# jakubbober/discrete-curvature-rewiring

Hardware: AMD Instinct MI355X
Metric: SDRF iterations/sec (higher is better)
Workload: dtype f64; 1 GPU; S100k: preferential-attachment graph N=100000 m=10 E=999900 (PCG64 seed 12345), Balanced Forman curvature, full recompute every iteration, remove_edges=True, tau=163.0, removal_bound=0.95; parallelism=single GPU

## Files before the change

discrete-curvature-rewiring_amd/csrc/dcr_bfc_h2.hip:

```cpp
#include <algorithm>
#include <climits>
#include <cstdio>
#include <cstdlib>
#include <cstring>
#include <vector>

#include "dcr_bfc_common.h"

namespace dcr {

constexpr unsigned H2_EMPTY = 0xFFFFFFFFu;
constexpr unsigned H2_NBR = 0x80000000u;
constexpr int H2_CLASSES = 5;
constexpr int H2_WB = 4;
__device__ inline unsigned h2_rec_t(int T, int deg) { return (unsigned)T | ((unsigned)deg << 16); }
static_assert(H2_MAXDEG < 65536, "record packing");
constexpr int H2_SMALL_DEG = 64;
#ifndef H2_Q
#define H2_Q 2
#endif
#ifndef H2_QL
#define H2_QL 2
#endif
constexpr int H2_QCAP = 128;
// ... 943 lines not shown
    int pln = sc->pln;
#pragma unroll 1
    while (true) {
        const int i = lcur + lane;
        const unsigned item = i < ls.n ? ls.items[i] : 0xFFFFFFFFu;
        const bool mine = i < ls.n && (int)(item >> 19) == bidx;
        const int cnt = __popcll(__ballot(mine));
        if (cnt == 0) break;
        const int s = (int)(item & 0x1FFFu), r = (int)((item >> 13) & 63u);
        const unsigned w = mine ? t.key[s] : 0u;
        h2_settle<L1, EXS>(t, sc, mine, mine ? s : -1, r, w, pln, tk, al, tbase);
        lcur += cnt;
        if (cnt < 64) break;
    }
    if (lane == 0) sc->pln = pln;
    h2_wave_sync();
}

__device__ inline void h2_batch_begin(const H2Tasks tk, H2Alloc &al, H2Scratch *sc, int k, int &tbase, int &trow, int rev = -1) {
    const int lane = threadIdx.x & 63;
    const unsigned long long below = (1ull << lane) - 1ull;
    sc->rowT[lane] = 0;
    sc->rowPos[lane] = 0;
    sc->rowMx[lane] = 0;
    sc->rowRev[lane] = rev;
    if (lane == 0) sc->pln = 0;
    int dummy_c, dummy_p;
    const unsigned long long rows = __ballot(k >= 0);
    if (!h2_pool_reserve(tk, al, __popcll(rows), 0, 0, tbase, dummy_c, dummy_p)) tbase = -1;
    trow = __popcll(rows & below);
    sc->trank[lane] = (unsigned char)trow;
    trow += tbase;
}

template <int L1, int EXS, bool PARTS>
__device__ inline void h2_batch_end(const View &g, const H2Tasks tk, H2Alloc &al, int u, int2 ru, int i, int k, int2 rk, int tbase,
                                    int trow, int part, const H2Tab t, H2Scratch *sc, uint4 *rec, const unsigned *items = nullptr,
                                    int ifrom = 0, int ito = 0) {
    const int lane = threadIdx.x & 63;
    int T = sc->rowT[lane], pos = sc->rowPos[lane], mx = sc->rowMx[lane];
    const int rev = sc->rowRev[lane];
    bool listed = tbase >= 0 && k >= 0 && T > 0 && pos > 0 && rev >= 0 && rev < g.cap_total;
    int ep;
    const int Pn = h2_prefix(listed ? T : 0, ep);
    int p0 = 0;
    if (Pn > 0) {
        int dummy_t, dummy_c;
        if (!h2_pool_reserve(tk, al, 0, 0, Pn, dummy_t, dummy_c, p0)) listed = false;
    }
    if (__ballot(listed) != 0ull) {
        const int pln = sc->pln;
        if (pln <= H2_PLCAP) {
            sc->poff[lane] = listed ? p0 + ep : -1;
            h2_wave_sync();
            for (int j = lane; j < pln; j += 64) {
                const int r = sc->plr[j];
                if (sc->poff[r] >= 0) tk.part[atomicAdd(&sc->poff[r], 1)] = (int32_t)sc->plt[j];
            }
            h2_wave_sync();
        } else if (items) {
            sc->poff[lane] = listed ? p0 + ep : -1;
            h2_wave_sync();
            for (int j = ifrom + lane; j < ito; j += 64) {
                const unsigned item = items[j];
                const int s2 = (int)(item & 0x1FFFu), r = (int)((item >> 13) & 63u);
                if ((h2_cnt_get(t.cnt, s2) & 0x8000u) && sc->poff[r] >= 0) tk.part[atomicAdd(&sc->poff[r], 1)] = (int32_t)t.key[s2];
            }
            h2_wave_sync();
        } else {
            const bool shortrow = listed && rk.y <= H2_SHORT_ROW;
            if (shortrow) h2_partners_short<L1, EXS>(g, tk, u, rk, p0 + ep, T, t);
            unsigned long long todo = __ballot(listed && !shortrow);
            while (todo) {
                const int l = __ffsll((long long)todo) - 1;
                todo &= todo - 1;
                const int2 rv = make_int2(__shfl(rk.x, l), __shfl(rk.y, l));
                h2_partners_of_row<L1, EXS>(g, tk, u, rv, __shfl(p0 + ep, l), __shfl(T, l), t);
            }
        }
    }
    if (tbase >= 0 && k >= 0) {
        tk.task[trow] = listed ? make_uint4((unsigned)(ru.x + i), (unsigned)(p0 + ep), (unsigned)T, (unsigned)u | tk.retry_flag)
                               : make_uint4(0u, 0u, H2_TASK_VOID, 0u);
    }
    if (listed) {
        pos = 0;
        mx = 0;
    }
    if (k >= 0) {
        const int64_t slot = (int64_t)ru.x + i;
        if (rev < 0 || rev >= g.cap_total) {
            row_ok(g, make_int2(-1, rev), 33, u, k);
        } else if (!PARTS) {
            rec[slot] = make_uint4((unsigned)pos, (unsigned)mx, h2_rec_t(T, ru.y), (unsigned)rev);
        } else {
            unsigned *r4 = reinterpret_cast<unsigned *>(rec + slot);
            if (pos) atomicAdd(&r4[0], (unsigned)pos);
            if (mx) atomicMax(&r4[1], (unsigned)mx);
            if (part == 0) {
                r4[2] = h2_rec_t(T, ru.y);
                r4[3] = (unsigned)rev;
            }
        }
    }
}

constexpr int H2_JOIN_MAXM = 256;
__device__ inline int h2_probe_partners(const H2EdgeSet es, int w, const int32_t *pt, int np);

template <int L1, int EXS, int NW>
__device__ inline bool h2_join_prepare(const View &g, const H2Tab t, int2 ru, const H2List &ls) {
    constexpr int NT = 64 * NW, PER = EXS / NT;
    static_assert(PER >= 2 && PER % 2 == 0, "a thread owns whole cursor words");
    static_assert(EXS / 2 <= (1 << L1) / 32, "the cursors fit B1");
    static_assert(NW * H2_ITEMS < 65536 && EXS <= 8192, "16-bit cursors, 13-bit slots");
    const int tid = (int)threadIdx.x, lane = tid & 63, wid = tid >> 6;
    unsigned *cur = t.b1;
    int n[PER], sum = 0, most = 0;
#pragma unroll
    for (int q = 0; q < PER; ++q) {
        const unsigned c16 = h2_cnt_get(t.cnt, tid * PER + q);
        n[q] = ((c16 & 0x8000u) || c16 < 2u) ? 0 : (int)c16;
        sum += n[q];
        most = n[q] > most ? n[q] : most;
    }
    if (__syncthreads_or(most > H2_JOIN_MAXM)) return false;
    int excl;
    const int wtot = h2_prefix(sum, excl);
    if (lane == 0) t.wsum[wid] = wtot;
    __syncthreads();
    int off = excl;
    for (int w = 0; w < wid; ++w) off += t.wsum[w];
#pragma unroll
    for (int q = 0; q < PER; q += 2) {
        const unsigned lo = (unsigned)off;
        off += n[q];
        const unsigned hi = (unsigned)off;
        off += n[q + 1];
        cur[(tid * PER + q) >> 1] = lo | (hi << 16);
    }
    __syncthreads();
    for (int base = 0; base < ls.n; base += 64) {
        const int j = base + lane;
        if (j >= ls.n) continue;
        const unsigned item = ls.items[j];
        const int s = (int)(item & 0x1FFFu), r = (int)((item >> 13) & 63u), b = (int)(item >> 19);
        const unsigned c16 = h2_cnt_get(t.cnt, s);
        if ((c16 & 0x8000u) || c16 < 2u) continue;
        const int row = (b * 64 + r) * NW + wid;
        if (row >= ru.y) {
            row_ok(g, make_int2(-1, row), 44, ru.y, (int)item);
            continue;
        }
        const int v = g.col[ru.x + row];
        const unsigned old = atomicAdd(&cur[s >> 1], 1u << ((s & 1) * 16));
        const int p = (int)((old >> ((s & 1) * 16)) & 0xFFFFu);
        if (p < NW * H2_ITEMS) ls.srt[p] = v;
        else row_ok(g, make_int2(-1, p), 45, s, (int)c16);
    }
    __syncthreads();
    return true;
}

template <int L1, int EXS, int NW, bool PARTS>
__device__ inline void h2_batch_join(const View &g, const H2Tasks tk, H2Alloc &al, int u, int2 ru, int i, int k, int2 rk, int part,
                                     const H2Tab t, H2Scratch *sc, uint4 *rec, const H2List &ls, int &lcur, int bidx, int rev) {
    const int lane = threadIdx.x & 63;
    sc->rowT[lane] = 0;
    sc->rowPos[lane] = 0;
    sc->rowMx[lane] = 0;
    sc->rowRev[lane] = rev;
    if (lane == 0) sc->pln = 0;
    h2_wave_sync();
    const int lfrom = lcur;
#pragma unroll 1
    while (true) {
        const int j = lcur + lane;
        const unsigned item = j < ls.n ? ls.items[j] : 0xFFFFFFFFu;
        const bool mine = j < ls.n && (int)(item >> 19) == bidx;
        const int cnt = __popcll(__ballot(mine));
        if (cnt == 0) break;
        if (mine && (h2_cnt_get(t.cnt, (int)(item & 0x1FFFu)) & 0x8000u)) atomicAdd(&sc->rowT[(item >> 13) & 63u], 1);
        lcur += cnt;
        if (cnt < 64) break;
    }
    h2_wave_sync();
    const unsigned *cur = t.b1;
#pragma unroll 1
    for (int base = lfrom; base < lcur; base += 64) {
        const int j = base + lane;
        const bool have = j < lcur;
        const unsigned item = have ? ls.items[j] : 0u;
        const int s = (int)(item & 0x1FFFu), r = (int)((item >> 13) & 63u);
        const int vr = __shfl(k, r);
        if (!have) continue;
        const unsigned c16 = h2_cnt_get(t.cnt, s);
        if (c16 & 0x8000u) continue;
        const int m = (int)(c16 & 0x7FFFu);
        int c = m - 1;
        if (c <= 0) continue;
        if (sc->rowT[r] > 0 && vr >= 0) {
            const int end = (int)((cur[s >> 1] >> ((s & 1) * 16)) & 0xFFFFu);
            if (end >= m && end <= NW * H2_ITEMS) {
                c -= h2_probe_partners(tk.es, vr, ls.srt + (end - m), m);
            } else {
                row_ok(g, make_int2(-1, end), 46, s, m);
                c = 0;
            }
        }
        if (c > 0) {
            atomicAdd(&sc->rowPos[r], 1);
            atomicMax(&sc->rowMx[r], c);
        }
    }
    h2_wave_sync();
    h2_batch_end<L1, EXS, PARTS>(g, tk, al, u, ru, i, k, rk, -1, 0, part, t, sc, rec);
}

template <int L1, int EXS, int NW, bool PARTS, int PHASE>
__device__ inline void h2_stream(const View &g, const H2Tasks tk, H2Alloc &al, int u, int2 ru, int part, int nparts,
                                 const H2Tab t, H2Scratch *sc, uint4 *rec, int k0, int2 rk0, H2List &ls) {
    const int lane = threadIdx.x & 63;
    const int wid = (int)(threadIdx.x >> 6);
    int qn = 0;
    int lcur = 0;
    if (PHASE == 0 && ru.y > 64 * NW * H2_REV_BATCHES) ls.over = true;
    for (int base = 0; base < ru.y; base += 64 * NW) {
        const int i = base + lane * NW + wid;
        int k = k0;
        int2 rk = rk0;
        if (base > 0) {
            k = -1;
            rk = make_int2(0, 0);
            if (i < ru.y) {
                k = g.col[ru.x + i];
                if (k >= 0 && k < g.n && k != u) {
                    rk = g.rowinfo[k];
                    if (!row_ok(g, rk, 32, k, u)) rk = make_int2(0, 0);
                } else {
                    k = -1;
                }
            }
        }
        const int np = rk.y > 0 ? ((rk.x + rk.y + 3) >> 2) - (rk.x >> 2) : 0;
        int poff_lane;
        const int P = h2_prefix(np, poff_lane);
        if (P == 0) continue;
        const int bidx = base / (64 * NW);
        int tbase = -1, trow = 0;
        if (PHASE == 2 && !ls.over) {
            if (ls.join) {
                h2_batch_join<L1, EXS, NW, PARTS>(g, tk, al, u, ru, i, k, rk, part, t, sc, rec, ls, lcur, bidx, ls.revs[bidx * 64 + lane]);
                h2_wave_sync();
                continue;
            }
            h2_batch_begin(tk, al, sc, k, tbase, trow, ls.revs[bidx * 64 + lane]);
            h2_wave_sync();
            const int lfrom = lcur;
            h2_settle_items<L1, EXS>(t, sc, ls, lcur, bidx, tk, al, tbase);
            h2_batch_end<L1, EXS, PARTS>(g, tk, al, u, ru, i, k, rk, tbase, trow, part, t, sc, rec, ls.items, lfrom, lcur);
            h2_wave_sync();
            continue;
        }
        if (PHASE == 0 && !ls.over) ls.revs[bidx * 64 + lane] = -1;
        sc->desc[lane] = rk;
        sc->poff[lane] = poff_lane;
        if (lane == 0) sc->poff[64] = P;
        if (PHASE == 2) h2_batch_begin(tk, al, sc, k, tbase, trow);
        h2_wave_sync();
        const bool listing = PHASE == 1 && !ls.over;
        auto flags = [&](const int4 w, unsigned vm, int r, int a) -> unsigned {
            const unsigned kk[4] = {(unsigned)w.x, (unsigned)w.y, (unsigned)w.z, (unsigned)w.w};
            const unsigned isu = h2_eq4(kk, (unsigned)u) & vm;
            if (PHASE == 2 && isu) sc->rowRev[r] = a + __ffs((int)isu) - 1;
            if (listing && isu) ls.revs[bidx * 64 + r] = a + __ffs((int)isu) - 1;
            unsigned valid = vm & ~isu;
            if (PARTS && PHASE != 2 && !listing) {
#pragma unroll
                for (int jj = 0; jj < 4; ++jj)
                    if (h2_part(kk[jj], nparts) != part) valid &= ~(1u << jj);
            }
            if (PHASE == 0) {
                h2_mark4<L1>(t.b1, t.b2, kk, valid);
                return 0u;
            }
            return h2_again4<L1>(t.b2, kk, valid);
        };
        h2_for_pieces_queued<(PARTS ? H2_QL : H2_Q)>(g.col, sc->desc, sc->poff, poff_lane, P, qn, flags,
                             [&](int idx, unsigned key, int r) {
                                 sc->qw[idx] = key;
                                 if (PHASE != 0) sc->qr[idx] = (unsigned char)r;
                                 if (PHASE == 1) sc->qb[idx] = (unsigned char)bidx;
                             },
                             [&]() { h2_drain<L1, EXS, PHASE, PARTS>(t, sc, qn, tk, al, tbase, ls, part, nparts); });
        if (PHASE == 2) {
            h2_drain<L1, EXS, PHASE, PARTS>(t, sc, qn, tk, al, tbase, ls, part, nparts);
            h2_batch_end<L1, EXS, PARTS>(g, tk, al, u, ru, i, k, rk, tbase, trow, part, t, sc, rec);
        }
        h2_wave_sync();
    }
    if (qn > 0) h2_drain<L1, EXS, PHASE, PARTS>(t, sc, qn, tk, al, -1, ls, part, nparts);
}

constexpr int H2_NPB = 12;
template <int L1, int EXS, int NW, bool PARTS>
__device__ inline bool h2_node_fast(const View &g, const H2Tasks tk, H2Alloc &al, int u, int2 ru, int part, int nparts,
                                    const H2Tab t, H2Scratch *sc, uint4 *rec, bool &ok, H2List &ls) {
    const int tid = (int)threadIdx.x, lane = tid & 63, wid = tid >> 6;
    constexpr int NT = 64 * NW, NP = H2_NPB;
    const unsigned long long below = (1ull << lane) - 1ull;
    if (ru.y > 64 * NW) return false;
    const int i = lane * NW + wid;
    int k = -1;
    int2 rk = make_int2(0, 0);
    if (i < ru.y) {
        k = g.col[ru.x + i];
        if (k >= 0 && k < g.n && k != u) {
            rk = g.rowinfo[k];
            if (!row_ok(g, rk, 32, k, u)) rk = make_int2(0, 0);
        } else {
            k = -1;
        }
    }
    const int np = rk.y > 0 ? ((rk.x + rk.y + 3) >> 2) - (rk.x >> 2) : 0;
    int poff_lane;
    const int P = h2_prefix(np, poff_lane);
    if (__syncthreads_or(P > 64 * NP)) return false;
    {
        uint4 *z = reinterpret_cast<uint4 *>(t.b1);
        constexpr int NZ = ((1 << L1) / 32 + (1 << (L1 - 2)) / 32) / 4;
        for (int j = tid; j < NZ; j += NT) z[j] = make_uint4(0u, 0u, 0u, 0u);
        uint4 *k4 = reinterpret_cast<uint4 *>(t.key);
        for (int j = tid; j < EXS / 4; j += NT) k4[j] = make_uint4(H2_EMPTY, H2_EMPTY, H2_EMPTY, H2_EMPTY);
        uint4 *c4 = reinterpret_cast<uint4 *>(t.cnt);
        for (int j = tid; j < EXS / 8; j += NT) c4[j] = make_uint4(0u, 0u, 0u, 0u);
        if (tid == 0) *t.full = 0;
    }
    sc->desc[lane] = rk;
    sc->poff[lane] = poff_lane;
    if (lane == 0) sc->poff[64] = P;
    h2_wave_sync();
    int4 w[NP];
    unsigned long long meta[NP];
#pragma unroll
    for (int q = 0; q < NP; ++q) {
        const int j = 64 * q + lane;
        w[q] = make_int4(0, 0, 0, 0);
        meta[q] = 0ull;
        const int jf = 64 * q, jl = jf + 63 < P ? jf + 63 : P - 1;
        if (jf >= P) continue;
        const int r = h2_piece_row(sc->poff, poff_lane, j < P ? j : jl, jf, jl);
        if (j < P) {
            const int2 d = sc->desc[r];
            const int a = (d.x & ~3) + 4 * (j - sc->poff[r]);
            w[q] = load_piece(g.col, a);
            meta[q] = (unsigned long long)h2_piece_mask(a, d.x, d.x + d.y) | ((unsigned long long)r << 8) | ((unsigned long long)(unsigned)a << 16);
        }
    }
    __syncthreads();
    if (k >= 0) {
        const int sl = h2_insert<EXS>(t.key, (unsigned)k);
        if (sl < 0) *t.full = 1;
        else h2_cnt_flag(t.cnt, sl);
        h2_seed<L1>(t.b1, t.b2, (unsigned)k);
    }
    __syncthreads();
#pragma unroll
    for (int q = 0; q < NP; ++q) {
        if (64 * q >= P) continue;
        const unsigned kk[4] = {(unsigned)w[q].x, (unsigned)w[q].y, (unsigned)w[q].z, (unsigned)w[q].w};
        unsigned valid = (unsigned)meta[q] & 0xFu & ~h2_eq4(kk, (unsigned)u);
        if (PARTS) {
#pragma unroll
            for (int jj = 0; jj < 4; ++jj)
                if (h2_part(kk[jj], nparts) != part) valid &= ~(1u << jj);
        }
        meta[q] |= (unsigned long long)valid << 4;
        h2_mark4<L1>(t.b1, t.b2, kk, valid);
    }
    __syncthreads();
    int qn = 0, tbase = -1, trow = 0;
    sc->rowRev[lane] = -1;
    h2_wave_sync();
    {
        unsigned fl[NP];
#pragma unroll
        for (int q = 0; q < NP; ++q) {
            fl[q] = 0u;
            if (64 * q >= P) continue;
            const unsigned kk[4] = {(unsigned)w[q].x, (unsigned)w[q].y, (unsigned)w[q].z, (unsigned)w[q].w};
            const unsigned valid = (unsigned)(meta[q] >> 4) & 0xFu;
            const unsigned isu = h2_eq4(kk, (unsigned)u) & (unsigned)meta[q] & 0xFu;
            if (isu) sc->rowRev[(int)((meta[q] >> 8) & 0xFFull)] = (int)(meta[q] >> 16) + __ffs((int)isu) - 1;
            fl[q] = h2_again4<L1>(t.b2, kk, valid);
        }
#pragma unroll 1
        while (true) {
            bool stop = false;
#pragma unroll
            for (int q = 0; q < NP; ++q) {
                if (64 * q >= P) continue;
                const unsigned kk[4] = {(unsigned)w[q].x, (unsigned)w[q].y, (unsigned)w[q].z, (unsigned)w[q].w};
#pragma unroll
                for (int jj = 0; jj < 4; ++jj) {
                    const bool p = (fl[q] >> jj) & 1u;
                    const unsigned long long m = __ballot(p);
                    if (m == 0ull) continue;
                    if (stop || qn + __popcll(m) > H2_QCAP) {
                        stop = true;
                        continue;
                    }
                    if (p) {
                        const int idx = qn + __popcll(m & below);
                        sc->qw[idx] = kk[jj];
                        sc->qr[idx] = (unsigned char)((meta[q] >> 8) & 0xFFull);
                        sc->qb[idx] = 0;
                        fl[q] &= ~(1u << jj);
                    }
                    qn += __popcll(m);
                }
            }
            if (qn > 0) h2_drain<L1, EXS, 1, PARTS>(t, sc, qn, tk, al, -1, ls, part, nparts);
            if (!stop) break;
        }
    }
    __syncthreads();
    ok = *t.full == 0;
    ls.join = !__syncthreads_or(ls.over) && ok;
    if (ls.join) ls.join = h2_join_prepare<L1, EXS, NW>(g, t, ru, ls);
    if (ls.join) {
        int lcur = 0;
        const int myrev = sc->rowRev[lane];
        h2_wave_sync();
        h2_batch_join<L1, EXS, NW, PARTS>(g, tk, al, u, ru, i, k, rk, part, t, sc, rec, ls, lcur, 0, myrev);
    } else if (ok) {
        if (tid == 0) atomicAdd(&tk.res->h2_fallback, 1);
        if (!ls.over) {
            int lcur = 0;
            const int myrev = sc->rowRev[lane];
            h2_wave_sync();
            h2_batch_begin(tk, al, sc, k, tbase, trow, myrev);
            h2_wave_sync();
            h2_settle_items<L1, EXS>(t, sc, ls, lcur, 0, tk, al, tbase);
            h2_batch_end<L1, EXS, PARTS>(g, tk, al, u, ru, i, k, rk, tbase, trow, part, t, sc, rec, ls.items, 0, lcur);
        } else {
            h2_stream<L1, EXS, NW, PARTS, 2>(g, tk, al, u, ru, part, nparts, t, sc, rec, k, rk, ls);
        }
    }
    __syncthreads();
    return true;
}

template <int L1, int EXS, int NW, bool PARTS>
__device__ inline bool h2_node(const View &g, const H2Tasks tk, H2Alloc &al, int u, int2 ru, int part, int nparts,
                               const H2Tab t, H2Scratch *sc, uint4 *rec, H2List &ls) {
    const int tid = (int)threadIdx.x;
    constexpr int NT = 64 * NW;
    if constexpr (!PARTS) {
        bool ok_fast = true;
        if (h2_node_fast<L1, EXS, NW, PARTS>(g, tk, al, u, ru, part, nparts, t, sc, rec, ok_fast, ls)) return ok_fast;
    }
    int k0 = -1;
    int2 rk0 = make_int2(0, 0);
    {
        const int i0 = (tid & 63) * NW + (tid >> 6);
        if (i0 < ru.y) {
            k0 = g.col[ru.x + i0];
            if (k0 >= 0 && k0 < g.n && k0 != u) {
                rk0 = g.rowinfo[k0];
                if (!row_ok(g, rk0, 32, k0, u)) rk0 = make_int2(0, 0);
            } else {
                k0 = -1;
            }
        }
    }
    {
        uint4 *z = reinterpret_cast<uint4 *>(t.b1);
        constexpr int NZ = ((1 << L1) / 32 + (1 << (L1 - 2)) / 32) / 4;
        for (int i = tid; i < NZ; i += NT) z[i] = make_uint4(0u, 0u, 0u, 0u);
        uint4 *k4 = reinterpret_cast<uint4 *>(t.key);
        for (int i = tid; i < EXS / 4; i += NT) k4[i] = make_uint4(H2_EMPTY, H2_EMPTY, H2_EMPTY, H2_EMPTY);
        uint4 *c4 = reinterpret_cast<uint4 *>(t.cnt);
        for (int i = tid; i < EXS / 8; i += NT) c4[i] = make_uint4(0u, 0u, 0u, 0u);
        if (tid == 0) *t.full = 0;
    }
    __syncthreads();
    for (int i = tid; i < ru.y; i += NT) {
        const int k = g.col[ru.x + i];
        if (k >= 0 && k < g.n && k != u) {
            const int s = h2_insert<EXS>(t.key, (unsigned)k);
            if (s < 0) *t.full = 1;
            else h2_cnt_flag(t.cnt, s);
            h2_seed<L1>(t.b1, t.b2, (unsigned)k);
        }
    }
    __syncthreads();
    h2_stream<L1, EXS, NW, PARTS, 0>(g, tk, al, u, ru, part, nparts, t, sc, rec, k0, rk0, ls);
    __syncthreads();
    h2_stream<L1, EXS, NW, PARTS, 1>(g, tk, al, u, ru, part, nparts, t, sc, rec, k0, rk0, ls);
    __syncthreads();
    const bool ok = *t.full == 0;
    ls.join = !__syncthreads_or(ls.over) && ok;
    if (ls.join) ls.join = h2_join_prepare<L1, EXS, NW>(g, t, ru, ls);
    if (!ls.join && ok && tid == 0) atomicAdd(&tk.res->h2_fallback, 1);
    if (ok) h2_stream<L1, EXS, NW, PARTS, 2>(g, tk, al, u, ru, part, nparts, t, sc, rec, k0, rk0, ls);
    __syncthreads();
    return ok;
}

template <int L1, int EXS, int NW, bool PARTS>
__global__ void __launch_bounds__(64 * NW) __attribute__((amdgpu_waves_per_eu(3))) k_h2_block(View g, H2Tasks tk, const int4 *units, const int32_t *count, int64_t unit_cap,
                                                       uint4 *rec, H2Retry rt, int is_retry) {
    __shared__ __attribute__((aligned(16))) unsigned bits[(1 << L1) / 32 + (1 << (L1 - 2)) / 32];
    __shared__ __attribute__((aligned(16))) unsigned key[EXS];
    __shared__ __attribute__((aligned(16))) unsigned cnt[EXS / 2];
    __shared__ H2Scratch sc_all[NW];
    __shared__ int full;
    __shared__ int wsum[NW];
    const int wid = threadIdx.x >> 6;
    const int total = *count;
    if (total < 0 || total > unit_cap) {
        row_ok(g, make_int2(-1, total), 37, 0, 0);
        return;
    }
    const H2Tab t{bits, bits + (1 << L1) / 32, key, cnt, &full, wsum};
    H2Alloc al;
    for (int64_t it = blockIdx.x; it < total; it += gridDim.x) {
        const int4 un = units[it];
        const int u = un.x;
        const int nparts = PARTS ? (int)((unsigned)un.y >> 16) : 1, part = PARTS ? (un.y & 0xFFFF) : 0;
        bool ok = u >= 0 && u < g.n && nparts >= 1 && part < nparts;
        int2 ru = make_int2(0, 0);
        if (ok) {
            ru = g.rowinfo[u];
            ok = row_ok(g, ru, 38, u, (int)it) && ru.y > 0 && ru.y <= H2_MAXDEG;
        }
        if (!ok) continue;
        H2List ls = h2_list_of(tk.lists, NW);
        const bool unit_ok = h2_node<L1, EXS, NW, PARTS>(g, tk, al, u, ru, part, nparts, t, &sc_all[wid], rec, ls);
        if (!unit_ok) {
            if (threadIdx.x == 0) {
                if (is_retry) {
                    rt.res->h2_status = 1;
                    atomicAdd(&rt.res->h2_failed[5], 1);
                } else {
                    h2_retry_push(rt, u, ru.y, PARTS ? 4 : 3);
                }
            }
        }
    }
    h2_void_candidates(tk, al.c_cur, al.c_end);
    h2_void_tasks(tk, al.t_cur, al.t_end);
}

__device__ inline int h2_probe_partners(const H2EdgeSet es, int w, const int32_t *pt, int np) {
    int found = 0;
    for (int j = 0; j < np; j += 8) {
        int tt[8];
#pragma unroll
        for (int q = 0; q < 8; ++q) tt[q] = j + q < np ? pt[j + q] : -1;
        unsigned long long key[8], k0[8], h[8];
        unsigned bw[8], bb[8];
#pragma unroll
        for (int q = 0; q < 8; ++q) {
            key[q] = h2_edge_key(w, tt[q] < 0 ? w : tt[q]);
            bb[q] = h2_bloom_bit(key[q], es.bloom_bits);
            bw[q] = es.bloom[bb[q] >> 5];
        }
#pragma unroll
        for (int q = 0; q < 8; ++q) {
            const bool maybe = tt[q] >= 0 && ((bw[q] >> (bb[q] & 31u)) & 1u);
            h[q] = h2_eset_slot(key[q], es.bits);
            k0[q] = maybe ? es.tab[h[q]] : H2_ESET_EMPTY;
        }
#pragma unroll
        for (int q = 0; q < 8; ++q) {
            bool hit = k0[q] == key[q];
            if (!hit && k0[q] != H2_ESET_EMPTY) hit = h2_eset_has(es, w, tt[q]);
            found += hit ? 1 : 0;
        }
    }
    return found;
}

__global__ void __launch_bounds__(256) k_h2_triangles(H2EdgeSet es, H2Tasks tk, uint4 *rec, const int32_t *status, int second) {
    const int cand_now = *tk.n_cand;
    const int first = second ? *tk.n_done : 0;
    const int total = cand_now < tk.cand_cap ? cand_now : (int)tk.cand_cap;
    if (!second && blockIdx.x == 0 && threadIdx.x == 0) *tk.n_done = cand_now;
    if (*status != 0) return;
    if (total <= first || first < 0) return;
    const int lane = threadIdx.x & 63;
    for (int64_t base = first + (((int64_t)blockIdx.x * 256 + threadIdx.x) & ~63ll); base < total; base += (int64_t)gridDim.x * 256) {
        const int64_t i = base + lane;
        int c = 0;
        unsigned slot = 0xFFFFFFFFu;
        if (i < total) {
            const int4 cd = tk.cand[i];
            const uint4 ts = (cd.z >= 0 && cd.z < tk.task_cap) ? tk.task[cd.z] : make_uint4(0u, 0u, H2_TASK_VOID, 0u);
            const bool skip = ts.z == H2_TASK_VOID || (!(ts.w & 0x80000000u) && ((unsigned)tk.weight[ts.w & 0x7FFFFFFFu] & 0x80000000u));
            if (!skip) {
                slot = ts.x;
                c = cd.y - h2_probe_partners(es, cd.x, tk.part + ts.y, (int)ts.z);
            }
        }
        const unsigned prev = (unsigned)__shfl_up((int)slot, 1);
        const bool head = lane == 0 || prev != slot;
        const unsigned long long heads = __ballot(head);
        const int seg = __popcll(heads & ((2ull << lane) - 1ull));
        int n = c > 0 ? 1 : 0, mx = c > 0 ? c : 0;
#pragma unroll
        for (int off = 1; off < 64; off <<= 1) {
            const int s2 = __shfl_up(seg, off), n2 = __shfl_up(n, off), m2 = __shfl_up(mx, off);
            if (lane >= off && s2 == seg) {
                n += n2;
                mx = m2 > mx ? m2 : mx;
            }
        }
        const bool tail = lane == 63 || ((heads >> (lane + 1)) & 1ull);
        if (tail && n > 0 && slot != 0xFFFFFFFFu) {
            unsigned *r4 = reinterpret_cast<unsigned *>(rec + slot);
            atomicAdd(&r4[0], (unsigned)n);
            atomicMax(&r4[1], (unsigned)mx);
        }
    }
}

__global__ void __launch_bounds__(256) k_h2_weight(View g, int32_t *weight) {
    const int64_t s = (int64_t)blockIdx.x * 256 + threadIdx.x;
    const int lane = threadIdx.x & 63;
    int u = -1, val = 0;
    if (s < g.cap_total) {
        const int us = g.slot_row[s];
        const int v = g.col[s];
        const bool uok = us >= 0 && us < g.n, vok = v >= 0 && v < g.n;
        const int2 ru = g.rowinfo[uok ? us : 0];
        const int dv = g.rowinfo[vok ? v : 0].y;
        if (uok) {
            u = us;
            if (vok && s >= ru.x && (int)(s - ru.x) < ru.y) val = dv;
        }
    }
#pragma unroll
    for (int off = 1; off < 64; off <<= 1) {
        const int t = __shfl_up(val, off), uu = __shfl_up(u, off);
        if (lane >= off && uu == u) val += t;
    }
    const int un = __shfl_down(u, 1);
    if (u >= 0 && val > 0 && (lane == 63 || un != u)) atomicAdd(&weight[u], val);
}

constexpr int H2_NB = H2_CLASSES * H2_WB;
__device__ inline void h2_clear_result(DevResult *res, int tid, int half, bool flags_cleared) {
    if (tid == 0 && flags_cleared) res->touched_n = 0;
    if (tid < 8) res->misc[tid] = 0;
    if (tid < H2_NB) {
        res->h2_bucket[half][tid] = 0;
        res->h2_fill[half][tid] = 0;
    }
    if (tid < H2_CLASSES) res->h2_count[tid] = 0;
    if (tid == 0) {
        res->h2_status = 0;
        res->h2_retry = 0;
        for (int p = 0; p < 2; ++p) res->h2_ntask[p] = res->h2_ncand[p] = res->h2_npart[p] = res->h2_ncand_done[p] = 0;
        for (int c = 0; c < 6; ++c) res->h2_failed[c] = 0;
        res->h2_fallback = 0;
        res->flag_too_big = 0;
    }
}
struct H2Lists {
    int4 *units[H2_CLASSES];
    int64_t cap[H2_CLASSES];
};
constexpr int H2_PLAN_THREADS = 1024;

__device__ inline void h2_classify(int d, int S, int &cls, int &wb, int &nparts) {
    nparts = 1;
    int lo = 0;
    if (d <= H2_SMALL_DEG && S <= h2_maxw(2)) {
        cls = S <= h2_maxw(0) ? 0 : S <= h2_maxw(1) ? 1 : 2;
        lo = cls == 0 ? 0 : h2_maxw(cls - 1);
        wb = (int)((int64_t)(S - lo) * H2_WB / (h2_maxw(cls) - lo + 1));
    } else if (S <= h2_maxw(3) && d + S / 4 <= h2_keycap(3)) {
        cls = 3;
        wb = S < 2048 ? 0 : S < 4096 ? 1 : S < 6144 ? 2 : 3;
    } else {
        cls = 4;
        nparts = h2_parts_for(d, S, false);
        wb = S < 16384 ? 0 : S < 32768 ? 1 : S < 65536 ? 2 : 3;
    }
    if (wb > H2_WB - 1) wb = H2_WB - 1;
    if (wb < 0) wb = 0;
}

template <int PHASE>
__global__ void __launch_bounds__(H2_PLAN_THREADS) k_h2_plan(View g, int32_t *weight, H2Lists L, DevResult *res, int parity, int head,
                                                             unsigned *dirty_words, int64_t n_dirty_words, uint4 *rec) {
    __shared__ int blk_count[H2_NB];
    __shared__ int blk_base[H2_NB];
    const int u = blockIdx.x * H2_PLAN_THREADS + threadIdx.x;
    const int lane = threadIdx.x & 63;
    if (threadIdx.x < H2_NB) blk_count[threadIdx.x] = 0;
    __syncthreads();
    int bkt = -1, cls = -1, wb = 0, nparts = 0;
    int2 ru = make_int2(0, 0);
    if (u < g.n) {
        ru = g.rowinfo[u];
        const int d = ru.y;
        const int wraw = weight[u];
        if (PHASE == 0 && wraw < 0) weight[u] = wraw & 0x7FFFFFFF;
        if (d > 0 && d <= H2_MAXDEG) {
            h2_classify(d, wraw & 0x7FFFFFFF, cls, wb, nparts);
            bkt = cls * H2_WB + wb;
        }
    }
    if (PHASE == 0 && head) {
        const int64_t stride = (int64_t)gridDim.x * H2_PLAN_THREADS;
        for (int64_t i = (int64_t)blockIdx.x * H2_PLAN_THREADS + threadIdx.x; i < n_dirty_words; i += stride) dirty_words[i] = 0u;
        if (blockIdx.x == 0) h2_clear_result(res, (int)threadIdx.x, 1 - parity, n_dirty_words > 0);
    }
    const int nunits = bkt < 0 ? 0 : nparts;
    int my_off = 0;
    for (int b = 0; b < H2_NB; ++b) {
        const unsigned long long m = __ballot(bkt == b);
        if (m == 0) continue;
        int incl = bkt == b ? nunits : 0;
        for (int off = 1; off < 64; off <<= 1) {
            const int t = __shfl_up(incl, off);
            if (lane >= off) incl += t;
        }
        const int tot = __shfl(incl, 63);
        int wave_off = 0;
        if (lane == 0) wave_off = atomicAdd(&blk_count[b], tot);
        wave_off = __shfl(wave_off, 0);
        if (bkt == b) my_off = wave_off + incl - nunits;
    }
    __syncthreads();
    if (threadIdx.x < H2_NB) {
        const int b = threadIdx.x, c = blk_count[b];
        if (PHASE == 0) {
            if (c) atomicAdd(&res->h2_bucket[parity][b], c);
        } else {
            int before = 0;
            for (int h = b + 1; h < H2_NB; ++h)
                if (h / H2_WB == b / H2_WB) before += res->h2_bucket[parity][h];
            blk_base[b] = before + (c ? atomicAdd(&res->h2_fill[parity][b], c) : 0);
        }
    }
    if (PHASE == 0) return;
    if (blockIdx.x == 0 && threadIdx.x >= 64 && threadIdx.x < 64 + H2_CLASSES) {
        const int c = (int)threadIdx.x - 64;
        int64_t tot = 0;
        for (int b = c * H2_WB; b < (c + 1) * H2_WB; ++b) tot += res->h2_bucket[parity][b];
        if (tot > (c == 0 ? L.cap[0] : c == 1 ? L.cap[1] : c == 2 ? L.cap[2] : c == 3 ? L.cap[3] : L.cap[4])) {
            res->h2_status = 1;
            tot = 0;
        }
        res->h2_count[c] = (int)tot;
    }
    __syncthreads();
    if (bkt >= 0) {
        const int64_t first = (int64_t)blk_base[bkt] + my_off;
        int4 *dst = cls == 0 ? L.units[0] : cls == 1 ? L.units[1] : cls == 2 ? L.units[2] : cls == 3 ? L.units[3] : L.units[4];
        const int64_t cap = cls == 0 ? L.cap[0] : cls == 1 ? L.cap[1] : cls == 2 ? L.cap[2] : cls == 3 ? L.cap[3] : L.cap[4];
        static_assert(H2_CLASSES == 5, "the selects above list the classes");
        if (nparts <= 65535 && first >= 0 && first + nunits <= cap) {
            for (int j = 0; j < nunits; ++j) dst[first + j] = make_int4(u, (nparts << 16) | j, ru.x, ru.y);
        } else if (nparts > 65535) {
            res->h2_status = 1;
        }
    }
    if (!head) return;
    const int64_t piece = (int64_t)((lane >> 3) * (H2_PLAN_THREADS / 64) + (int)(threadIdx.x >> 6)) * gridDim.x + blockIdx.x;
    const int64_t z = piece * 8 + (lane & 7);
    int2 rz = make_int2(0, 0);
    bool is_split = false;
    if (z < g.n) {
        rz = g.rowinfo[z];
        if (rz.y > 0 && rz.y <= H2_MAXDEG) {
            int zc, zb, zp;
            h2_classify(rz.y, weight[z] & 0x7FFFFFFF, zc, zb, zp);
            is_split = zc == 4;
        }
    }
    unsigned long long split = __ballot(is_split);
    while (split) {
        const int src = __ffsll((long long)split) - 1;
        split &= split - 1ull;
        const int2 rs = make_int2(__shfl(rz.x, src), __shfl(rz.y, src));
        if (!row_ok(g, rs, 42, __shfl((int)z, src), -1)) continue;
        for (int i = lane; i < rs.y; i += 64) rec[(int64_t)rs.x + i] = make_uint4(0u, 0u, 0u, 0u);
    }
}

__global__ void __launch_bounds__(256) k_h2_clear(DevResult *res, int32_t *weight, int64_t n, unsigned *dirty_words, int64_t n_dirty_words) {
    for (int64_t i = (int64_t)blockIdx.x * 256 + threadIdx.x; i < n; i += (int64_t)gridDim.x * 256) weight[i] = 0;
    for (int64_t i = (int64_t)blockIdx.x * 256 + threadIdx.x; i < n_dirty_words; i += (int64_t)gridDim.x * 256) dirty_words[i] = 0u;
    if (blockIdx.x != 0) return;
    h2_clear_result(res, (int)threadIdx.x, 0, n_dirty_words > 0);
    h2_clear_result(res, (int)threadIdx.x, 1, n_dirty_words > 0);
}

__global__ void __launch_bounds__(256) k_h2_retry_zero(View g, const int4 *units, const int32_t *count, int64_t unit_cap, uint4 *rec) {
    const int total = *count;
    if (total <= 0 || total > unit_cap) return;
    for (int64_t it = blockIdx.x; it < total; it += gridDim.x) {
        const int4 un = units[it];
        if ((un.y & 0xFFFF) != 0 || un.x < 0 || un.x >= g.n) continue;
        const int2 ru = g.rowinfo[un.x];
        if (!row_ok(g, ru, 42, un.x, (int)it)) continue;
        for (int i = threadIdx.x; i < ru.y; i += 256) rec[(int64_t)ru.x + i] = make_uint4(0u, 0u, 0u, 0u);
    }
}

#ifndef H2_FINAL_Q
#define H2_FINAL_Q 1
#endif
#ifndef H2_FINAL_BLOCKS
#define H2_FINAL_BLOCKS 1024
#endif
__global__ void __launch_bounds__(256) k_h2_final(View g, const uint4 *rec, double *curv, const int32_t *status, Ext *part_min,
                                                  Ext *part_max, const int32_t *retry_count, int when, const int32_t *fallback_count,
                                                  int tri_stage) {
    if (when == 0 && *retry_count > 0) {
        if (blockIdx.x == 0 && threadIdx.x == 0) atomicCAS(const_cast<int32_t *>(status), 0, 3);
        return;
    }
    if (tri_stage == 0 && *fallback_count > 0) {
        if (blockIdx.x == 0 && threadIdx.x == 0) atomicCAS(const_cast<int32_t *>(status), 0, 4);
        return;
    }
    double lo_v = 0.0, hi_v = 0.0;
    int lo_s = -1, hi_s = -1;
    const bool live = *status == 0;
    const int64_t stride = (int64_t)gridDim.x * 256;
    constexpr int Q = H2_FINAL_Q;
    for (int64_t s0 = (int64_t)blockIdx.x * 256 + threadIdx.x; live && s0 < g.cap_total; s0 += Q * stride) {
        int u[Q], v[Q];
        uint4 a[Q];
        bool want[Q];
#pragma unroll
        for (int q = 0; q < Q; ++q) {
            const int64_t s = s0 + q * stride;
            const bool in = s < g.cap_total;
            u[q] = in ? g.slot_row[s] : -1;
            v[q] = in ? g.col[s] : -1;
            a[q] = in ? rec[s] : make_uint4(0u, 0u, 0u, 0u);
        }
        int2 ru[Q];
        int dv[Q], rcol[Q], rrow[Q];
        uint4 b[Q];
// ... 306 lines not shown
```

Before: 1119 iterations/sec.

## Software-pipeline unit and neighbour-head loads across block-loop iterations in H2 kernel

Prefetches the next two work units, plus the first-hop neighbour index and row info for the next unit, while the current unit is processed. Row offset and degree carried inside the unit record let the kernel skip a dependent rowinfo load. It also uses readfirstlane to keep unit fields uniform in scalar registers. The goal is to hide the global-memory latency of the dependent col/rowinfo chain at the start of each unit, at the cost of extra live registers and reliance on units carrying valid row info in z/w.

```diff
diff --git a/discrete-curvature-rewiring_amd/csrc/dcr_bfc_h2.hip b/discrete-curvature-rewiring_amd/csrc/dcr_bfc_h2.hip
--- a/discrete-curvature-rewiring_amd/csrc/dcr_bfc_h2.hip
+++ b/discrete-curvature-rewiring_amd/csrc/dcr_bfc_h2.hip
@@ -1269,26 +1269,34 @@
     if (qn > 0) h2_drain<L1, EXS, PHASE, PARTS>(t, sc, qn, tk, al, -1, ls, part, nparts);
 }
 
+template <int NW>
+__device__ inline int h2_head_k(const View &g, int2 ru) {
+    const int i0 = (int)(threadIdx.x & 63) * NW + (int)(threadIdx.x >> 6);
+    return i0 < ru.y ? g.col[ru.x + i0] : -1;
+}
+__device__ inline int2 h2_head_rk(const View &g, int u, int k) {
+    return (k >= 0 && k < g.n && k != u) ? g.rowinfo[k] : make_int2(0, 0);
+}
+template <int NW>
+__device__ inline void h2_head_check(const View &g, int u, int2 ru, int &k, int2 &rk) {
+    const int i0 = (int)(threadIdx.x & 63) * NW + (int)(threadIdx.x >> 6);
+    if (i0 >= ru.y || k < 0 || k >= g.n || k == u) {
+        k = -1;
+        rk = make_int2(0, 0);
+    } else if (!row_ok(g, rk, 32, k, u)) {
+        rk = make_int2(0, 0);
+    }
+}
+
 constexpr int H2_NPB = 12;
-template <int L1, int EXS, int NW, bool PARTS>
+template <int L1, int EXS, int NW, bool PARTS, typename Mid>
 __device__ inline bool h2_node_fast(const View &g, const H2Tasks tk, H2Alloc &al, int u, int2 ru, int part, int nparts,
-                                    const H2Tab t, H2Scratch *sc, uint4 *rec, bool &ok, H2List &ls) {
+                                    const H2Tab t, H2Scratch *sc, uint4 *rec, bool &ok, H2List &ls, int k, int2 rk, Mid mid) {
     const int tid = (int)threadIdx.x, lane = tid & 63, wid = tid >> 6;
     constexpr int NT = 64 * NW, NP = H2_NPB;
     const unsigned long long below = (1ull << lane) - 1ull;
     if (ru.y > 64 * NW) return false;
     const int i = lane * NW + wid;
-    int k = -1;
-    int2 rk = make_int2(0, 0);
-    if (i < ru.y) {
-        k = g.col[ru.x + i];
-        if (k >= 0 && k < g.n && k != u) {
-            rk = g.rowinfo[k];
-            if (!row_ok(g, rk, 32, k, u)) rk = make_int2(0, 0);
-        } else {
-            k = -1;
-        }
-    }
     const int np = rk.y > 0 ? ((rk.x + rk.y + 3) >> 2) - (rk.x >> 2) : 0;
     int poff_lane;
     const int P = h2_prefix(np, poff_lane);
@@ -1345,6 +1353,7 @@
         meta[q] |= (unsigned long long)valid << 4;
         h2_mark4<L1>(t.b1, t.b2, kk, valid);
     }
+    mid();
     __syncthreads();
     int qn = 0, tbase = -1, trow = 0;
     sc->rowRev[lane] = -1;
@@ -1418,28 +1427,14 @@
     return true;
 }
 
-template <int L1, int EXS, int NW, bool PARTS>
+template <int L1, int EXS, int NW, bool PARTS, typename Mid>
 __device__ inline bool h2_node(const View &g, const H2Tasks tk, H2Alloc &al, int u, int2 ru, int part, int nparts,
-                               const H2Tab t, H2Scratch *sc, uint4 *rec, H2List &ls) {
+                               const H2Tab t, H2Scratch *sc, uint4 *rec, H2List &ls, int k0, int2 rk0, Mid mid) {
     const int tid = (int)threadIdx.x;
     constexpr int NT = 64 * NW;
     if constexpr (!PARTS) {
         bool ok_fast = true;
-        if (h2_node_fast<L1, EXS, NW, PARTS>(g, tk, al, u, ru, part, nparts, t, sc, rec, ok_fast, ls)) return ok_fast;
-    }
-    int k0 = -1;
-    int2 rk0 = make_int2(0, 0);
-    {
-        const int i0 = (tid & 63) * NW + (tid >> 6);
-        if (i0 < ru.y) {
-            k0 = g.col[ru.x + i0];
-            if (k0 >= 0 && k0 < g.n && k0 != u) {
-                rk0 = g.rowinfo[k0];
-                if (!row_ok(g, rk0, 32, k0, u)) rk0 = make_int2(0, 0);
-            } else {
-                k0 = -1;
-            }
-        }
+        if (h2_node_fast<L1, EXS, NW, PARTS>(g, tk, al, u, ru, part, nparts, t, sc, rec, ok_fast, ls, k0, rk0, mid)) return ok_fast;
     }
     {
         uint4 *z = reinterpret_cast<uint4 *>(t.b1);
@@ -1463,6 +1458,7 @@
     }
     __syncthreads();
     h2_stream<L1, EXS, NW, PARTS, 0>(g, tk, al, u, ru, part, nparts, t, sc, rec, k0, rk0, ls);
+    mid();
     __syncthreads();
     h2_stream<L1, EXS, NW, PARTS, 1>(g, tk, al, u, ru, part, nparts, t, sc, rec, k0, rk0, ls);
     __syncthreads();
@@ -1492,28 +1488,85 @@
     }
     const H2Tab t{bits, bits + (1 << L1) / 32, key, cnt, &full, wsum};
     H2Alloc al;
-    for (int64_t it = blockIdx.x; it < total; it += gridDim.x) {
-        const int4 un = units[it];
+    const int64_t stride = gridDim.x;
+    const int4 none = make_int4(-1, 0, 0, 0);
+    auto unit_at = [&](int64_t j) {
+        if (j >= total) return none;
+        const int4 v = units[j];
+        if constexpr (PARTS) return v;
+        else return make_int4(__builtin_amdgcn_readfirstlane(v.x), __builtin_amdgcn_readfirstlane(v.y), __builtin_amdgcn_readfirstlane(v.z),
+                         __builtin_amdgcn_readfirstlane(v.w));
+    };
+    auto carries_row = [&](const int4 v) {
+        return v.x >= 0 && v.x < g.n && v.w > 0 && v.w <= H2_MAXDEG && v.z >= 0 && (int64_t)v.z + v.w <= g.cap_total;
+    };
+    int4 un = none, un1 = none;
+    int k = -1, k1 = -1;
+    int2 rk = make_int2(0, 0);
+    if constexpr (!PARTS) {
+        un = unit_at(blockIdx.x);
+        un1 = unit_at(blockIdx.x + stride);
+        if (carries_row(un)) {
+            k = h2_head_k<NW>(g, make_int2(un.z, un.w));
+            rk = h2_head_rk(g, un.x, k);
+        }
+        if (carries_row(un1)) k1 = h2_head_k<NW>(g, make_int2(un1.z, un1.w));
+    }
+    for (int64_t it = blockIdx.x; it < total; it += stride) {
+        int4 un2 = none;
+        if constexpr (PARTS) un = unit_at(it);
+        else un2 = unit_at(it + 2 * stride);
+        int2 rk1 = make_int2(0, 0);
+        auto mid = [&]() {
+            if constexpr (!PARTS) rk1 = h2_head_rk(g, un1.x, k1);
+        };
         const int u = un.x;
         const int nparts = PARTS ? (int)((unsigned)un.y >> 16) : 1, part = PARTS ? (un.y & 0xFFFF) : 0;
+        const bool carried = un.w > 0;
         bool ok = u >= 0 && u < g.n && nparts >= 1 && part < nparts;
         int2 ru = make_int2(0, 0);
         if (ok) {
-            ru = g.rowinfo[u];
+            ru = carried ? make_int2(un.z, un.w) : g.rowinfo[u];
             ok = row_ok(g, ru, 38, u, (int)it) && ru.y > 0 && ru.y <= H2_MAXDEG;
         }
-        if (!ok) continue;
-        H2List ls = h2_list_of(tk.lists, NW);
-        const bool unit_ok = h2_node<L1, EXS, NW, PARTS>(g, tk, al, u, ru, part, nparts, t, &sc_all[wid], rec, ls);
-        if (!unit_ok) {
-            if (threadIdx.x == 0) {
-                if (is_retry) {
-                    rt.res->h2_status = 1;
-                    atomicAdd(&rt.res->h2_failed[5], 1);
-                } else {
-                    h2_retry_push(rt, u, ru.y, PARTS ? 4 : 3);
+        if (ok) {
+            if (PARTS || !carried) {
+                const int i0 = (int)(threadIdx.x & 63) * NW + (int)(threadIdx.x >> 6);
+                k = -1;
+                rk = make_int2(0, 0);
+                if (i0 < ru.y) {
+                    k = g.col[ru.x + i0];
+                    if (k >= 0 && k < g.n && k != u) {
+                        rk = g.rowinfo[k];
+                        if (!row_ok(g, rk, 32, k, u)) rk = make_int2(0, 0);
+                    } else {
+                        k = -1;
+                    }
                 }
-            }
+            } else {
+                h2_head_check<NW>(g, u, ru, k, rk);
+            }
+            H2List ls = h2_list_of(tk.lists, NW);
+            const bool unit_ok = h2_node<L1, EXS, NW, PARTS>(g, tk, al, u, ru, part, nparts, t, &sc_all[wid], rec, ls, k, rk, mid);
+            if (!unit_ok) {
+                if (threadIdx.x == 0) {
+                    if (is_retry) {
+                        rt.res->h2_status = 1;
+                        atomicAdd(&rt.res->h2_failed[5], 1);
+                    } else {
+                        h2_retry_push(rt, u, ru.y, PARTS ? 4 : 3);
+                    }
+                }
+            }
+        } else {
+            mid();
+        }
+        if constexpr (!PARTS) {
+            un = un1;
+            k = k1;
+            rk = rk1;
+            un1 = un2;
+            k1 = carries_row(un1) ? h2_head_k<NW>(g, make_int2(un1.z, un1.w)) : -1;
         }
     }
     h2_void_candidates(tk, al.c_cur, al.c_end);
```

Result: no change. 1114 iterations/sec (-0.4%).
